# jungmannlab/picasso

Hardware: AMD Instinct MI355X
Metric: localizations/sec (7x7 ROI, MLE) (higher is better)
Workload: dtype f32+f64; 1 GPU; 10000-frame 512x512 uint16 simulated DNA-PAINT movie per GPU, 1001675 spots per GPU, 7x7 ROI MLE (sigmaxy), identify+cut+fit+table resident in HBM; frames=10000, height=512, width=512, box=7, max_it=100, localizations_total=1001675, mle_mode=refit, refit_spots_rank0=7346, frame_ranges_in_flight=2, all_gather=none

## Files before the change

picasso_amd/csrc/fit_common.h:

```cpp
#pragma once
#include <math.h>

#include "pmi_common.h"

namespace pmi {

#ifndef FIT_WAVES_N
#define FIT_WAVES_N 4
#endif
constexpr int FIT_WAVES = FIT_WAVES_N;
constexpr int FIT_NT = FIT_WAVES * PMI_WAVE;
constexpr int FIT_MAXPIX = PMI_MAX_BOX * PMI_MAX_BOX;

struct ConstDiv { float g, r; int fast; };
inline ConstDiv make_const_div(float g)
{
    ConstDiv c;
    c.g = g;
    c.r = (float)(1.0 / (double)g);
    c.fast = (g == g) && fabsf(g) > 1e-15f && fabsf(g) < 1e15f;
    if (g == 1.0f) c.fast = 2;
    return c;
}
__device__ __forceinline__ float div_const(float x, const ConstDiv &c)
// ... 29 lines not shown
    }
}

struct FitParams {
    const float *spots;
    float *spots_out;
    const void *movie;
    const int32_t *frame, *y, *x;
    int dtype;
    int64_t Y, X;
    float baseline, sensitivity, gain;
    ConstDiv gdiv;
    int64_t N;
    const int64_t *d_n;
    int box;
    int libm_glibc;
    double eps;
    int max_it;
    float *thetas, *crlbs, *loglik;
    int32_t *iterations;
    unsigned long long *queue;
    unsigned *strict_queue;
    int64_t first;
    double *fisher;
    float eps_lo, eps_hi;
    int32_t *flag_list;
    unsigned *flag_count;
    unsigned *flag_reasons;
    const int32_t *final_list;
    const unsigned *final_list_n;
    unsigned char *refit_mark;
    float *ng_io;
    unsigned char *accept;
    int crop_y0, crop_x0, crop_cy, crop_cx;
    double min_ng;
    const int32_t *alist;
    const unsigned *alist_n;
    int32_t *alist_out;
    unsigned *alist_blk_out;
};
enum : unsigned { FLAG_MARGIN = 1u, FLAG_CURVATURE = 2u, FLAG_NARROW = 4u, FLAG_SWING = 8u, FLAG_WILD = 16u, FLAG_SLOW = 32u, FLAG_UNSTABLE = 64u };
constexpr int FLAG_REASONS = 7;
constexpr double FIT_UNSTABLE_LMAX = 1.9;
constexpr int FISHER_STRIDE = 21;
enum { FIT_STAGE_NEWTON = 1, FIT_STAGE_FINAL = 2, FIT_STAGE_INIT_ONLY = 4, FIT_STAGE_ITERATE_ONLY = 8 };
constexpr int FIT_SLOW_ITERATIONS = 64;
#ifndef PMI_MARGIN_GROWTH
#define PMI_MARGIN_GROWTH 0.0625f
#endif
constexpr float FIT_MARGIN_GROWTH = PMI_MARGIN_GROWTH;
constexpr float FIT_NARROW_SIGMA = 0.5f;
constexpr float FIT_WOBBLE_RATIO = 0.9f;
constexpr float FIT_WOBBLE_FLOOR = 1.9073486e-6f;
constexpr int FIT_WOBBLE_RUN = 3;
constexpr int FIT_WOBBLE_LATE = 9;
constexpr float FIT_TOP_FLAG = 16.0f;

template <int CTRL, int ROW_MASK = 0xf>
__device__ __forceinline__ float dpp_f(float v)
{
    return __builtin_bit_cast(float, __builtin_amdgcn_update_dpp(0, __builtin_bit_cast(int, v), CTRL, ROW_MASK, 0xf, false));
}
__device__ __forceinline__ float wave_sum(float v)
{
    v += dpp_f<0xB1>(v);
    v += dpp_f<0x4E>(v);
    v += dpp_f<0x141>(v);
    v += dpp_f<0x140>(v);
    v += dpp_f<0x142, 0xA>(v);
    v += dpp_f<0x143, 0xC>(v);
    return __builtin_bit_cast(float, __builtin_amdgcn_readlane(__builtin_bit_cast(int, v), 63));
}
template <int CTRL, int ROW_MASK = 0xf>
__device__ __forceinline__ double dpp_d(double v)
{
    long long b = __builtin_bit_cast(long long, v);
    int lo = (int)(b & 0xffffffffLL), hi = (int)(b >> 32);
    lo = __builtin_amdgcn_update_dpp(0, lo, CTRL, ROW_MASK, 0xf, false);
// ... 68 lines not shown
```

picasso_amd/csrc/gaussmle.hip:

```cpp
#include <algorithm>
#include <cmath>
#include <cstdlib>
#include <cstring>
#include <vector>

#include "fit_common.h"

namespace pmi {

__device__ __forceinline__ unsigned borderline(float D, int kk, float eps_lo, float eps_hi)
{
    const float wide = fmaxf(1.0f, (float)(kk - 1) * FIT_MARGIN_GROWTH);
    const float epsf = 0.5f * (eps_lo + eps_hi), epsm = 0.5f * (eps_hi - eps_lo) * wide;
    return ((D >= epsf - epsm && D < epsf + epsm) ? FLAG_MARGIN : 0u) | (kk > FIT_SLOW_ITERATIONS ? FLAG_SLOW : 0u);
}
struct StepHistory { float prev, prev2, wprev; int run; };
__device__ __forceinline__ bool wobbles(float st, float value, int kk, StepHistory &h)
{
    const float w = kk >= 3 ? (st - 2.0f * h.prev) + h.prev2 : 0.0f;
    const bool wob = w * h.wprev < 0.0f && fabsf(w) > FIT_WOBBLE_RATIO * fabsf(h.wprev) && fabsf(w) > FIT_WOBBLE_FLOOR * fabsf(value);
    h.run = wob ? h.run + 1 : 0;
    h.wprev = w; h.prev2 = h.prev; h.prev = st;
    return h.run >= FIT_WOBBLE_RUN || (h.run >= 2 && kk >= FIT_WOBBLE_LATE);
}
// ... 266 lines not shown
{
    double A[36], V[36];
    bool nonfinite = false;
    for (int i = 0; i < NP * NP; i++) { A[i] = Min[i]; if (!isfinite(A[i])) nonfinite = true; }
    if (nonfinite) { for (int i = 0; i < NP; i++) diag[i] = NAN; return; }
    for (int i = 0; i < NP; i++) for (int j = 0; j < NP; j++) V[i * NP + j] = (i == j) ? 1.0 : 0.0;
    for (int sweep = 0; sweep < 60; sweep++) {
        double off = 0.0;
        for (int a = 0; a < NP; a++) for (int b = a + 1; b < NP; b++) off += A[a * NP + b] * A[a * NP + b];
        if (off == 0.0) break;
        for (int a = 0; a < NP; a++)
            for (int b = a + 1; b < NP; b++) {
                double apq = A[a * NP + b];
                if (apq == 0.0) continue;
                double tau = (A[b * NP + b] - A[a * NP + a]) / (2.0 * apq);
                double tt = (tau >= 0 ? 1.0 : -1.0) / (fabs(tau) + sqrt(1.0 + tau * tau));
                double c = 1.0 / sqrt(1.0 + tt * tt), s = tt * c;
                for (int k = 0; k < NP; k++) { double x = A[k * NP + a], y = A[k * NP + b]; A[k * NP + a] = c * x - s * y; A[k * NP + b] = s * x + c * y; }
                for (int k = 0; k < NP; k++) { double x = A[a * NP + k], y = A[b * NP + k]; A[a * NP + k] = c * x - s * y; A[b * NP + k] = s * x + c * y; }
                for (int k = 0; k < NP; k++) { double x = V[k * NP + a], y = V[k * NP + b]; V[k * NP + a] = c * x - s * y; V[k * NP + b] = s * x + c * y; }
            }
    }
    double smax = 0.0;
    for (int i = 0; i < NP; i++) smax = fmax(smax, fabs(A[i * NP + i]));
    const double cutoff = 1e-15 * smax;
    for (int i = 0; i < NP; i++) {
        double acc = 0.0;
        for (int k = 0; k < NP; k++) { double lam = A[k * NP + k]; if (fabs(lam) > cutoff) acc += V[i * NP + k] * V[i * NP + k] / lam; }
        diag[i] = acc;
    }
}

template <int NP>
__global__ __launch_bounds__(256) void crlb_kernel(const double *__restrict__ fisher, int64_t first, int64_t N,
                                                   const int64_t *__restrict__ d_n, float *__restrict__ crlbs,
                                                   const int32_t *__restrict__ list, const unsigned *__restrict__ list_n,
                                                   int32_t *__restrict__ unstable, unsigned *__restrict__ unstable_n,
                                                   unsigned *__restrict__ reasons, const unsigned char *__restrict__ refit_mark,
                                                   const unsigned char *__restrict__ accept)
{
    int64_t n = N;
    if (d_n) { int64_t dn = *d_n; n = dn < n ? dn : n; }
    int64_t t = (int64_t)blockIdx.x * blockDim.x + threadIdx.x;
    int64_t sidx = first + t;
    if (list) {
        if (t >= (int64_t)*list_n) return;
        sidx = (int64_t)list[t];
        t = sidx - first;
    } else if (sidx >= n) return;
    else if (accept && !accept[sidx]) return;
    const double *f = fisher + t * FISHER_STRIDE;
    double M[36];
    {
        int e = 0;
#pragma unroll
        for (int k = 0; k < NP; k++)
#pragma unroll
            for (int l = k; l < NP; l++) { const double v = f[e++]; M[k * NP + l] = v; M[l * NP + k] = v; }
    }
    if (unstable && !(refit_mark && refit_mark[t])) {
        double dinv[NP], v[NP], lam = 0.0;
        bool ok = true;
#pragma unroll
        for (int i = 0; i < NP; i++) { const double m = M[i * NP + i]; ok = ok && m > 0.0 && m < 1e300; dinv[i] = 1.0 / sqrt(m); v[i] = 1.0 + 0.125 * (double)i; }
        if (ok) {
            double C[NP * NP], C2[NP * NP], t8 = 0.0;
#pragma unroll
            for (int i = 0; i < NP; i++)
#pragma unroll
                for (int k = 0; k < NP; k++) C[i * NP + k] = M[i * NP + k] * dinv[i] * dinv[k];
#pragma unroll
            for (int i = 0; i < NP; i++)
#pragma unroll
                for (int k = i; k < NP; k++) {
                    double a = 0.0;
#pragma unroll
                    for (int q = 0; q < NP; q++) a += C[i * NP + q] * C[q * NP + k];
                    C2[i * NP + k] = a; C2[k * NP + i] = a;
                }
#pragma unroll
            for (int i = 0; i < NP; i++)
#pragma unroll
                for (int k = i; k < NP; k++) {
// ... 43 lines not shown
            if (c == i) { D[i] = a; rD[i] = 1.0 / a; if (!(a > 0.0)) bad = true; }
            else L[i * NP + c] = a * rD[c];
        }
    }
    double Li[36];
#pragma unroll
    for (int i = 0; i < NP; i++)
#pragma unroll
        for (int c = 0; c < NP; c++) Li[i * NP + c] = (i == c) ? 1.0 : 0.0;
#pragma unroll
    for (int c = 0; c < NP; c++)
#pragma unroll
        for (int i = c + 1; i < NP; i++) {
            double a = 0.0;
#pragma unroll
            for (int k = c; k < i; k++) a -= L[i * NP + k] * Li[k * NP + c];
            Li[i * NP + c] = a;
        }
    double trInv = 0.0;
#pragma unroll
    for (int i = 0; i < NP; i++) {
        double a = 0.0;
#pragma unroll
        for (int k = i; k < NP; k++) a += Li[k * NP + i] * Li[k * NP + i] * rD[k];
        diag[i] = a;
        trInv += a;
    }
    if (!(trM * trInv < 1e12)) bad = true;
    if (bad) pinv_diag_jacobi<NP>(M, diag);
    float *co = crlbs + sidx * 6;
#pragma unroll
    for (int l = 0; l < NP; l++) co[l] = (float)diag[l];
    if (NP == 5) co[5] = (float)diag[4];
}

template <int NP, bool FROM_MOVIE>
static void launch_fit_ppl(int ppl, dim3 grid, hipStream_t s, const FitParams &p, int stages)
{
    switch (ppl) {
    case 1: hipLaunchKernelGGL((mle_fit_kernel<NP, 1, FROM_MOVIE>), grid, dim3(FIT_NT), 0, s, p, stages); break;
    case 2: hipLaunchKernelGGL((mle_fit_kernel<NP, 2, FROM_MOVIE>), grid, dim3(FIT_NT), 0, s, p, stages); break;
    case 3: hipLaunchKernelGGL((mle_fit_kernel<NP, 3, FROM_MOVIE>), grid, dim3(FIT_NT), 0, s, p, stages); break;
    case 4: hipLaunchKernelGGL((mle_fit_kernel<NP, 4, FROM_MOVIE>), grid, dim3(FIT_NT), 0, s, p, stages); break;
    case 5: hipLaunchKernelGGL((mle_fit_kernel<NP, 5, FROM_MOVIE>), grid, dim3(FIT_NT), 0, s, p, stages); break;
    case 6: hipLaunchKernelGGL((mle_fit_kernel<NP, 6, FROM_MOVIE>), grid, dim3(FIT_NT), 0, s, p, stages); break;
    default: hipLaunchKernelGGL((mle_fit_kernel<NP, 7, FROM_MOVIE>), grid, dim3(FIT_NT), 0, s, p, stages); break;
    }
}


bool launch_fit_g8(const FitParams &p, int method, bool from_movie, int cu_count, float *state, int stages, hipStream_t s);
void launch_fit_strict(const FitParams &p, int method, bool from_movie, const int32_t *list, const unsigned *list_n,
                       int64_t max_items, int cu_count, hipStream_t s);

constexpr int64_t FIT_BATCH = 1 << 22;
constexpr int ACC_BLOCK = 1024;
__global__ __launch_bounds__(256) void accept_count_kernel(const unsigned char *__restrict__ accept, int64_t first, int64_t N,
                                                           const int64_t *__restrict__ d_n, unsigned *__restrict__ blk_cnt)
{
    int64_t n = N;
    if (d_n) { const int64_t dn = *d_n; n = dn < n ? dn : n; }
    __shared__ unsigned s_c[4];
    const int64_t base = first + (int64_t)blockIdx.x * ACC_BLOCK;
    unsigned c = 0;
#pragma unroll
    for (int q = 0; q < ACC_BLOCK / 256; q++) {
        const int64_t sp = base + q * 256 + threadIdx.x;
        c += (unsigned)__popcll(__ballot(sp < n && accept[sp] != 0));
    }
    if ((threadIdx.x & 63) == 0) s_c[threadIdx.x >> 6] = c;
    __syncthreads();
    if (threadIdx.x == 0) blk_cnt[blockIdx.x] = s_c[0] + s_c[1] + s_c[2] + s_c[3];
}
__global__ __launch_bounds__(1024) void accept_scan_kernel(unsigned *__restrict__ blk, int nblk, unsigned *__restrict__ total)
{
    __shared__ unsigned s_w[16];
    __shared__ unsigned s_carry;
    if (threadIdx.x == 0) s_carry = 0;
    __syncthreads();
    const int lane = threadIdx.x & 63, w = threadIdx.x >> 6;
    for (int b0 = 0; b0 < nblk; b0 += 1024) {
        const int i = b0 + (int)threadIdx.x;
        const unsigned v = i < nblk ? blk[i] : 0u;
        unsigned inc = v;
#pragma unroll
        for (int off = 1; off < 64; off <<= 1) { const unsigned t = __shfl_up(inc, off); if (lane >= off) inc += t; }
        if (lane == 63) s_w[w] = inc;
        __syncthreads();
        unsigned before = s_carry;
// ... 4 lines not shown
        __syncthreads();
    }
    if (threadIdx.x == 0) *total = s_carry;
}
__global__ __launch_bounds__(256) void accept_write_kernel(const unsigned char *__restrict__ accept, int64_t first, int64_t N,
                                                           const int64_t *__restrict__ d_n, const unsigned *__restrict__ blk_off,
                                                           int32_t *__restrict__ alist)
{
    int64_t n = N;
    if (d_n) { const int64_t dn = *d_n; n = dn < n ? dn : n; }
    __shared__ unsigned s_c[ACC_BLOCK / 64];
    const int64_t base = first + (int64_t)blockIdx.x * ACC_BLOCK;
    const int lane = threadIdx.x & 63, w = threadIdx.x >> 6;
    unsigned long long bal[ACC_BLOCK / 256];
#pragma unroll
    for (int q = 0; q < ACC_BLOCK / 256; q++) {
        const int64_t sp = base + q * 256 + threadIdx.x;
        bal[q] = __ballot(sp < n && accept[sp] != 0);
        if (lane == 0) s_c[q * 4 + w] = (unsigned)__popcll(bal[q]);
    }
    __syncthreads();
    const unsigned off0 = blk_off[blockIdx.x];
#pragma unroll
    for (int q = 0; q < ACC_BLOCK / 256; q++) {
        if ((bal[q] >> lane) & 1ull) {
            unsigned off = off0;
            for (int k = 0; k < q * 4 + w; k++) off += s_c[k];
            off += (unsigned)__popcll(bal[q] & ((1ull << lane) - 1ull));
            alist[off] = (int32_t)(base + q * 256 + threadIdx.x);
        }
    }
}
static int build_accept_list(const unsigned char *accept, int64_t first, int64_t N, const int64_t *d_n, unsigned *blk,
                             int32_t *alist, hipStream_t s)
{
    const int64_t count = N - first;
    const int nblk = (int)((count + ACC_BLOCK - 1) / ACC_BLOCK);
    hipLaunchKernelGGL(accept_count_kernel, dim3((unsigned)nblk), dim3(256), 0, s, accept, first, N, d_n, blk);
    hipLaunchKernelGGL(accept_scan_kernel, dim3(1), dim3(1024), 0, s, blk, nblk, blk + nblk);
    hipLaunchKernelGGL(accept_write_kernel, dim3((unsigned)nblk), dim3(256), 0, s, accept, first, N, d_n, (const unsigned *)blk, alist);
    PMI_HIP(hipGetLastError());
    return PMI_OK;
}

static int g_mle_mode = PMI_MLE_REFIT;
static double g_mle_margin = 0.001;
static int g_mle_libm = PMI_LIBM_AUTO;
static thread_local LastFitStats g_mle_stats;

__global__ void zero_words_kernel(unsigned *__restrict__ a, int na, unsigned *__restrict__ b, int nb)
{
    for (int i = threadIdx.x; i < na; i += blockDim.x) a[i] = 0u;
    for (int i = threadIdx.x; i < nb; i += blockDim.x) b[i] = 0u;
}

__global__ void flag_stats_kernel(const unsigned *__restrict__ flag_counts, int64_t nb, unsigned *__restrict__ stats)
{
    unsigned total = 0;
    for (int64_t b = 0; b < nb; b++) total += flag_counts[b];
    stats[0] = total;
}

static int mle_mode_now()
{
    static const char *env = getenv("PMI_MLE_MODE");
    if (env) {
        if (!strcmp(env, "fast")) return PMI_MLE_FAST;
        if (!strcmp(env, "strict")) return PMI_MLE_STRICT;
        if (!strcmp(env, "refit")) return PMI_MLE_REFIT;
    }
    return g_mle_mode;
}
static int mle_libm_now()
{
    static const char *env = getenv("PMI_MLE_LIBM");
    if (env) {
        if (!strcmp(env, "auto")) return PMI_LIBM_AUTO;
        if (!strcmp(env, "glibc")) return PMI_LIBM_GLIBC;
        if (!strcmp(env, "device")) return PMI_LIBM_DEVICE;
    }
    return g_mle_libm;
}

int fit_impl(FitParams p, int method, bool from_movie, int range, hipStream_t s)
{
    if (p.box < 3 || p.box > PMI_MAX_BOX || (p.box & 1) == 0) { set_error("box must be odd, 3..%d (got %d)", PMI_MAX_BOX, p.box); return PMI_ERR_ARG; }
    if (method != PMI_MLE_SIGMA && method != PMI_MLE_SIGMAXY) { set_error("Method not available."); return PMI_ERR_ARG; }
    if (p.N < 0) { set_error("negative N"); return PMI_ERR_ARG; }
    if (p.N == 0) return PMI_OK;
    if (p.N > 0x7fffffffLL) { set_error("too many spots for one call"); return PMI_ERR_ARG; }
    const int g_cu_count = device_cu_count();
    const int mode = mle_mode_now();
    const int64_t BATCH = FIT_BATCH;
    const int64_t nb = (p.N + BATCH - 1) / BATCH;
    void *ptr = nullptr, *fptr = nullptr;
    int rc;
    if ((rc = scratch(SCR_FIT, (size_t)nb * 40 + 64, &ptr)) != PMI_OK) return rc;
    const size_t per_batch = (size_t)std::min<int64_t>(p.N, BATCH);
    const size_t acc_blocks = (per_batch + ACC_BLOCK - 1) / ACC_BLOCK + 2;
    if ((rc = scratch(SCR_STAGE_D, per_batch * (FISHER_STRIDE * sizeof(double) + 12 * sizeof(float) + 3 * sizeof(int32_t) + 1) + acc_blocks * sizeof(unsigned) + 32, &fptr)) != PMI_OK) return rc;
    float *state = reinterpret_cast<float *>((char *)fptr + per_batch * FISHER_STRIDE * sizeof(double));
    int32_t *flag_list = reinterpret_cast<int32_t *>(state + per_batch * 12);
    int32_t *unstable_list = flag_list + per_batch;
    int32_t *acc_list = unstable_list + per_batch;
    unsigned *acc_blk = reinterpret_cast<unsigned *>(acc_list + per_batch);
    unsigned char *refit_mark = reinterpret_cast<unsigned char *>(acc_blk + acc_blocks);
    unsigned long long *queues = (unsigned long long *)ptr;
    unsigned *flag_counts = (unsigned *)(queues + 3 * nb);
    unsigned *strict_queues = flag_counts + 2 * nb;
    void *sptr = nullptr;
    if ((rc = scratch(SCR_STATS, 64, &sptr)) != PMI_OK) return rc;
    unsigned *stats = (unsigned *)sptr;
    hipLaunchKernelGGL(zero_words_kernel, dim3(1), dim3(256), 0, s, (unsigned *)ptr, (int)(nb * 10), stats, 16);
    p.flag_reasons = stats + 1;
    p.fisher = (double *)fptr;
    const int libm = mle_libm_now();
    const bool libm_all = libm != PMI_LIBM_DEVICE;
    p.libm_glibc = libm == PMI_LIBM_GLIBC || (libm == PMI_LIBM_AUTO && p.box <= 5);
    static const char *menv = tuning_env("PMI_MLE_MARGIN");
    const double margin = menv ? atof(menv) : g_mle_margin;
    const double ulp = ldexp(1.0, (int)floor(log2(std::max(1.0, p.box / 2.0))) - 23);
    const double margin_abs = std::max(p.eps * margin, 4.0 * ulp);
    p.eps_lo = (float)(p.eps - margin_abs);
    p.eps_hi = (float)(p.eps + margin_abs);
    const int ppl = (p.box * p.box + 63) / 64;
    const int64_t Ntotal = p.N;
    ScopedKernelTimer tm(s, &g_last_times.fit_ms);
    static const bool force_wave_per_spot = tuning_env("PMI_FIT_WAVE_PER_SPOT") != nullptr;
    const bool g8 = !force_wave_per_spot && p.box <= 15;
    float *cut = nullptr;
    static const bool no_keep = tuning_env("PMI_MLE_NO_KEEP") != nullptr;
    if (g8 && from_movie && mode != PMI_MLE_STRICT && !no_keep) {
        void *cptr = nullptr;
        if ((rc = scratch(SCR_STAGE_C, per_batch * (size_t)(p.box * p.box) * sizeof(float), &cptr)) != PMI_OK) return rc;
        cut = (float *)cptr;
    }
    p.spots_out = nullptr;
    if (p.ng_io && !(g8 && from_movie && cut)) { set_error("deferred exact stage outside the row-per-lane fit"); return PMI_ERR_ARG; }
    for (int64_t bi = 0; bi < nb; bi++) {
        p.first = bi * BATCH;
        p.N = std::min<int64_t>(Ntotal, p.first + BATCH);
        p.flag_list = mode == PMI_MLE_REFIT ? flag_list : nullptr;
        p.flag_count = flag_counts + bi;
        p.strict_queue = strict_queues + bi;
        p.refit_mark = mode == PMI_MLE_REFIT ? refit_mark : nullptr;
        if (p.refit_mark && !g8) PMI_HIP(hipMemsetAsync(refit_mark, 0, (size_t)(p.N - p.first), s));
        const int64_t count = p.N - p.first;
        const int64_t blocks = std::min<int64_t>((count + FIT_WAVES - 1) / FIT_WAVES, (int64_t)g_cu_count * 8);
        const dim3 grid((unsigned)std::max<int64_t>(blocks, 1));
        auto wave_per_spot = [&](int stages) {
            p.queue = queues + 3 * bi + (stages == FIT_STAGE_FINAL ? (p.final_list ? 2 : 1) : 0);
            if (method == PMI_MLE_SIGMAXY) {
                if (from_movie) launch_fit_ppl<6, true>(ppl, grid, s, p, stages); else launch_fit_ppl<6, false>(ppl, grid, s, p, stages);
            } else {
                if (from_movie) launch_fit_ppl<5, true>(ppl, grid, s, p, stages); else launch_fit_ppl<5, false>(ppl, grid, s, p, stages);
            }
        };
        if (mode != PMI_MLE_STRICT && g8 && from_movie && cut) {
            FitParams pi = p;
            pi.spots_out = cut;
            launch_fit_g8(pi, method, true, g_cu_count, state, FIT_STAGE_INIT_ONLY, s);
            PMI_HIP(hipGetLastError());
            FitParams q = p;
            q.spots = cut - p.first * (int64_t)(p.box * p.box);
            if (p.ng_io) {
                int32_t *al = nb == 1 && p.alist_out ? p.alist_out : acc_list;
                unsigned *ab = nb == 1 && p.alist_out ? p.alist_blk_out : acc_blk;
                if ((rc = build_accept_list(p.accept, p.first, p.N, p.d_n, ab, al, s)) != PMI_OK) return rc;
                q.alist = al;
                q.alist_n = ab + (count + ACC_BLOCK - 1) / ACC_BLOCK;
            }
            launch_fit_g8(q, method, false, g_cu_count, state, FIT_STAGE_ITERATE_ONLY, s);
            PMI_HIP(hipGetLastError());
            if (mode == PMI_MLE_REFIT)
                launch_fit_strict(q, method, false, flag_list, q.flag_count, count, g_cu_count, s);
            PMI_HIP(hipGetLastError());
            launch_fit_g8(q, method, false, g_cu_count, state, FIT_STAGE_FINAL, s);
        } else {
        if (mode == PMI_MLE_STRICT) {
            FitParams ps = p;
            ps.libm_glibc = libm_all;
            launch_fit_strict(ps, method, from_movie, nullptr, nullptr, count, g_cu_count, s);
        } else {
            if (g8) launch_fit_g8(p, method, from_movie, g_cu_count, state, FIT_STAGE_NEWTON, s);
            else wave_per_spot(FIT_STAGE_NEWTON);
            PMI_HIP(hipGetLastError());
            if (mode == PMI_MLE_REFIT)
                launch_fit_strict(p, method, from_movie, flag_list, p.flag_count, count, g_cu_count, s);
        }
        PMI_HIP(hipGetLastError());
        if (g8) launch_fit_g8(p, method, from_movie, g_cu_count, state, FIT_STAGE_FINAL, s);
        else wave_per_spot(FIT_STAGE_FINAL);
        }
        PMI_HIP(hipGetLastError());
        const unsigned cb = (unsigned)((count + 255) / 256);
        unsigned *unstable_n = flag_counts + nb + bi;
        auto crlb = [&](const int32_t *list, const unsigned *list_n, int32_t *out, unsigned *out_n) {
            if (method == PMI_MLE_SIGMAXY)
                hipLaunchKernelGGL((crlb_kernel<6>), dim3(cb), dim3(256), 0, s, p.fisher, p.first, p.N, p.d_n, p.crlbs, list, list_n, out, out_n, p.flag_reasons, p.refit_mark, p.accept);
            else
                hipLaunchKernelGGL((crlb_kernel<5>), dim3(cb), dim3(256), 0, s, p.fisher, p.first, p.N, p.d_n, p.crlbs, list, list_n, out, out_n, p.flag_reasons, p.refit_mark, p.accept);
        };
        const bool second = mode == PMI_MLE_REFIT;
        crlb(nullptr, nullptr, second ? unstable_list : nullptr, second ? unstable_n : nullptr);
        PMI_HIP(hipGetLastError());
        if (second) {
            FitParams r = p;
            r.strict_queue = strict_queues + nb + bi;
            if (cut) { r.spots = cut - p.first * (int64_t)(p.box * p.box); }
            const bool r_movie = cut ? false : from_movie;
            launch_fit_strict(r, method, r_movie, unstable_list, unstable_n, count, g_cu_count, s);
            PMI_HIP(hipGetLastError());
            r.final_list = unstable_list; r.final_list_n = unstable_n;
            if (g8) launch_fit_g8(r, method, r_movie, g_cu_count, state, FIT_STAGE_FINAL, s);
            else {
                FitParams keep = p;
                p = r;
                wave_per_spot(FIT_STAGE_FINAL);
                p = keep;
            }
            PMI_HIP(hipGetLastError());
            crlb(unstable_list, unstable_n, nullptr, nullptr);
            PMI_HIP(hipGetLastError());
        }
    }
    hipLaunchKernelGGL(flag_stats_kernel, dim3(1), dim3(1), 0, s, flag_counts, mode == PMI_MLE_REFIT ? 2 * nb : 0, stats);
    PMI_HIP(hipGetLastError());
    if ((rc = g_mle_stats.record(0, range, stats, s)) != PMI_OK) return rc;
    tm.stop();
    return PMI_OK;
}

static int read_last_stats(unsigned (&h)[16], hipStream_t s)
{
    if (g_mle_stats.valid()) PMI_HIP(hipStreamSynchronize(s));
    return g_mle_stats.read(h);
}

__global__ void cut_spots_kernel(const void *__restrict__ movie, int dtype, int64_t Y, int64_t X,
                                 const int32_t *__restrict__ frame, const int32_t *__restrict__ y,
                                 const int32_t *__restrict__ x, int64_t N, const int64_t *__restrict__ d_n,
                                 int box, float baseline, float sensitivity, ConstDiv gdiv, float *__restrict__ spots)
{
    int64_t n = N;
    if (d_n) { int64_t dn = *d_n; n = dn < n ? dn : n; }
    const int npix = box * box, h = box / 2;
    int64_t total = n * npix;
    for (int64_t t = (int64_t)blockIdx.x * blockDim.x + threadIdx.x; t < total; t += (int64_t)gridDim.x * blockDim.x) {
        int64_t i = t / npix;
        int q = (int)(t - i * npix);
        int a = q / box, c = q - a * box;
        float raw = load_movie_px(movie, dtype, ((int64_t)frame[i] * Y + (y[i] - h + a)) * X + (x[i] - h + c));
        spots[t] = div_const((raw - baseline) * sensitivity, gdiv);
    }
}
// ... 315 lines not shown
```

picasso_amd/csrc/gaussmle_g8.hip:

```cpp
#include <algorithm>

#include "fit_common.h"
#include "ng_common.h"

namespace pmi {

__device__ __forceinline__ float sum8(float v)
{
    v += dpp_f<0xB1>(v);
    v += dpp_f<0x4E>(v);
    v += dpp_f<0x141>(v);
    return v;
}
__device__ __forceinline__ float min8(float v)
{
    v = fminf(v, dpp_f<0xB1>(v));
    v = fminf(v, dpp_f<0x4E>(v));
    v = fminf(v, dpp_f<0x141>(v));
    return v;
}
__device__ __forceinline__ double sum8_d(double v)
{
    v += dpp_d<0xB1>(v);
    v += dpp_d<0x4E>(v);
// ... 437 lines not shown
                    for (int c = 0; c < W; c++) { nbt[c] = nb[c]; nbt[(W - 1) * W + c] = nb2[c]; }
                }
                __builtin_amdgcn_wave_barrier();
                __threadfence_block();
                const float vc = nbt[(H + 1) * W + (H + 1)];
                bool fm = true;
                if (rowok) {
#pragma unroll
                    for (int l = 0; l < B; l++) {
                        const float o = nb[l + 1];
                        const bool before = j < H || (j == H && l < H);
                        const bool centre = j == H && l == H;
                        fm = fm && (centre || (before ? vc > o : vc >= o));
                        const float gy = sub_rn(nbt[(j + 2) * W + l + 1], nbt[j * W + l + 1]);
                        const float gx = sub_rn(nb[l + 2], nb[l]);
                        terms[j * B + l] = add_rn(mul_rn(gy, uy[l]), mul_rn(gx, ux[l]));
                    }
                }
                __builtin_amdgcn_wave_barrier();
                __threadfence_block();
                float ng = 0.0f;
#pragma unroll
                for (int q = 0; q < B * B; q++)
                    if (q != H * B + H) ng = add_rn(ng, terms[q]);
                const unsigned long long gm = (GS == 64 ? ~0ull : ((1ull << GS) - 1ull)) << (lane & ~(GS - 1));
                const bool first_max = (__ballot(fm) & gm) == gm;
                if (need) {
                    keep = first_max && (double)ng > p.min_ng;
                    if (j == 0) p.ng_io[sidx] = ng;
                }
                __builtin_amdgcn_wave_barrier();
            }
            if (spot_ok && j == 0) p.accept[sidx] = keep ? 1 : 0;
        }
    }
    if (!loaded) load_row<B, FROM_MOVIE>(p, sidx, j, spot_ok && rowok, d);
    if (FROM_MOVIE && p.spots_out && spot_ok && rowok && keep) {
        float *o = p.spots_out + (sidx - p.first) * (B * B) + j * B;
#pragma unroll
        for (int i = 0; i < B; i++) o[i] = d[i];
    }

    double ps = 0.0, px = 0.0;
#pragma unroll
    for (int i = 0; i < B; i++) { ps += (double)d[i]; px += (double)d[i] * (double)i; }
    double sum = gsum_d<GS>(ps), sx_ = gsum_d<GS>(px), sy_ = gsum_d<GS>(ps * (double)j);
    float fmin_l = INFINITY;
    {
        double t3[B];
#pragma unroll
        for (int i = 0; i < B; i++) {
            double a = (double)d[i];
            if (i > 0) a = (double)d[i - 1] + a;
            if (i + 1 < B) a += (double)d[i + 1];
            t3[i] = a;
        }
        const bool up = j > 0, dn = j + 1 < B;
        const int nrow = 1 + (up ? 1 : 0) + (dn ? 1 : 0);
        const double n2 = (double)(nrow * 2), n3 = (double)(nrow * 3);
        const double r2 = 1.0 / n2, r3 = 1.0 / n3;
#pragma unroll
        for (int i = 0; i < B; i++) {
            const double a = from_prev_d(t3[i]), c = from_next_d(t3[i]);
            double tot = t3[i];
            if (up) tot = a + tot;
            if (dn) tot += c;
// ... 107 lines not shown
                    sidx = p.alist ? (int64_t)p.alist[cand] : cand;
                    const float4 *si = reinterpret_cast<const float4 *>(state + (sidx - p.first) * 12);
                    const float4 s0 = si[0], s1 = si[1], s2 = si[2];
                    th[0] = s0.x; th[1] = s0.y; th[2] = s0.z; th[3] = s0.w; th[4] = s1.x; th[5] = s1.y;
                    ms[0] = s1.z; ms[1] = s1.w; ms[2] = s2.x; ms[3] = s2.y; ms[4] = s2.z; ms[5] = s2.w;
                    load_row<B, FROM_MOVIE>(p, sidx, j, rowok, d);
                    role = make_role<NP, B>(th, ms, j);
                    kk = 0;
                    flags = 0u;
                    active = p.max_it > 0;
                    if (!active && j == 0) {
                        float *to = p.thetas + sidx * 6;
#pragma unroll
                        for (int l = 0; l < 5; l++) to[l] = th[l];
                        to[5] = NP == 6 ? th[5] : th[4];
                        p.iterations[sidx] = 0;
                        sidx = -1;
                    }
                }
            }
            next += __popcll(want);
            if (!__any(active)) {
                if (next >= end) break;
                continue;
            }
        } else if (!any_active) {
            break;
        }
        active = newton_step<NP, B>(d, th, role, xs, j, rowok, active, kk, p.eps, p.max_it, p.eps_lo, p.eps_hi, flags);
    }
}

template <int NP, int B, bool FROM_MOVIE>
__global__ __launch_bounds__(FIT_NT) void g8_final_kernel(FitParams p)
{
    constexpr int GS = GroupOf<B>::GS, NSPW = 64 / GS;
    __shared__ __attribute__((aligned(16))) double s_x[FIT_WAVES][NSPW][GS * 7];
    const int lane = threadIdx.x & 63, wid = threadIdx.x >> 6;
    const int g = lane / GS, j = lane & (GS - 1);
    const bool rowok = j < B;
    const float jf = (float)j;
    int64_t n = p.N;
    if (p.d_n) { int64_t dn = *p.d_n; n = dn < n ? dn : n; }
    int64_t sidx = p.first + ((int64_t)blockIdx.x * FIT_WAVES + wid) * NSPW + g;
    bool spot_ok = sidx < n;
    if (p.final_list) {
        const int64_t w0 = ((int64_t)blockIdx.x * FIT_WAVES + wid) * NSPW, items = (int64_t)*p.final_list_n;
        if (__builtin_amdgcn_readfirstlane((int)(w0 >= items))) return;
        spot_ok = w0 + g < items;
        sidx = spot_ok ? (int64_t)p.final_list[w0 + g] : p.first;
    } else if (__builtin_amdgcn_readfirstlane((int)(p.first + ((int64_t)blockIdx.x * FIT_WAVES + wid) * NSPW >= n))) return;
    else if (p.accept) spot_ok = spot_ok && p.accept[sidx] != 0;

    float d[B], th[6];
    load_row<B, FROM_MOVIE>(p, sidx, j, spot_ok && rowok, d);
#pragma unroll
    for (int l = 0; l < 6; l++) th[l] = spot_ok ? p.thetas[sidx * 6 + l] : 1.f;
    double *red = &s_x[wid][g][0];
    float *cols = reinterpret_cast<float *>(red);
    const float sgy = NP == 6 ? th[5] : th[4];
    const BTerms tx = boundary_terms(jf, th[0], th[4]);
    const BTerms ty = boundary_terms(jf, th[1], sgy);
    {
        float4 *c = reinterpret_cast<float4 *>(cols + j * 12);
        c[0] = make_float4(tx.A * tx.A, tx.A * tx.E, tx.A, tx.A * tx.S);
        c[1] = make_float4(tx.E * tx.E, tx.E, tx.E * tx.S, 1.0f);
        c[2] = make_float4(tx.S, tx.S * tx.S, 0.f, 0.f);
    }
    __builtin_amdgcn_wave_barrier();
    __threadfence_block();
    double T[10];
#pragma unroll
    for (int e = 0; e < 10; e++) T[e] = 0.0;
    float ll_loc = 0.f;
    const float N_ = th[2];
    const float NEy = N_ * ty.E;
#pragma unroll
    for (int i = 0; i < B; i++) {
        const float4 *c = reinterpret_cast<const float4 *>(cols + i * 12);
        const float4 c0 = c[0], c1 = c[1];
        const float2 c2 = *reinterpret_cast<const float2 *>(cols + i * 12 + 8);
        const float model = NEy * c1.y + th[3];
        if (rowok) {
            const double md = (double)model;
            double inv = (double)rcp_f32(model);
            inv = inv * (2.0 - md * inv);
            inv = inv * (2.0 - md * inv);
            T[0] += (double)c0.x * inv; T[1] += (double)c0.y * inv; T[2] += (double)c0.z * inv; T[3] += (double)c0.w * inv;
            T[4] += (double)c1.x * inv; T[5] += (double)c1.y * inv; T[6] += (double)c1.z * inv; T[7] += inv;
            T[8] += (double)c2.x * inv; T[9] += (double)c2.y * inv;
            if (model > 0.f) {
// ... 28 lines not shown
    constexpr int NE_ = NP * (NP + 1) / 2;
    double mine[3] = {0.0, 0.0, 0.0};
#pragma unroll
    for (int r0 = 0; r0 < 21; r0 += 7) {
        if (r0 < NE_) {
#pragma unroll
            for (int e = 0; e < 7; e++) red[j * 7 + e] = Mloc[r0 + e];
            __builtin_amdgcn_wave_barrier();
            __threadfence_block();
#pragma unroll
            for (int t = 0; t < 3; t++) {
                const int e = j + GS * t - r0;
                if (e >= 0 && e < 7) {
                    double acc = 0.0;
#pragma unroll
                    for (int r = 0; r < B; r++) acc += red[r * 7 + e];
                    mine[t] = acc;
                }
            }
            __builtin_amdgcn_wave_barrier();
        }
    }
    double *fo = p.fisher + (sidx - p.first) * FISHER_STRIDE;
    if (spot_ok) {
#pragma unroll
        for (int t = 0; t < 3; t++)
            if (j + GS * t < NE_) fo[j + GS * t] = mine[t];
    }
    const float ll = gsum<GS>(ll_loc);
    if (spot_ok && j == 0) p.loglik[sidx] = ll;
}

template <int NP, int B, bool FROM_MOVIE>
static void launch_g8(const FitParams &p, float *state, int cu_count, int stages, hipStream_t s)
{
    constexpr int NSPW = 64 / GroupOf<B>::GS;
    const int64_t count = p.N - p.first;
    const int64_t waves = (count + NSPW - 1) / NSPW;
    const dim3 flat((unsigned)((waves + FIT_WAVES - 1) / FIT_WAVES));
    const int64_t pw = std::max<int64_t>(1, std::min<int64_t>((int64_t)cu_count * 24, (count + 63) / 64));
    const dim3 pers((unsigned)((pw + FIT_WAVES - 1) / FIT_WAVES));
    if (stages & (FIT_STAGE_NEWTON | FIT_STAGE_INIT_ONLY))
        hipLaunchKernelGGL((g8_init_kernel<NP, B, FROM_MOVIE>), flat, dim3(FIT_NT), 0, s, p, state);
    if (stages & (FIT_STAGE_NEWTON | FIT_STAGE_ITERATE_ONLY))
        hipLaunchKernelGGL((g8_iterate_kernel<NP, B, FROM_MOVIE>), pers, dim3(FIT_NT), 0, s, p, (const float *)state);
    if (stages & FIT_STAGE_FINAL)
        hipLaunchKernelGGL((g8_final_kernel<NP, B, FROM_MOVIE>), flat, dim3(FIT_NT), 0, s, p);
}

template <int NP, bool FROM_MOVIE>
static void launch_g8_box(const FitParams &p, float *state, int cu_count, int stages, hipStream_t s)
{
    switch (p.box) {
    case 3: launch_g8<NP, 3, FROM_MOVIE>(p, state, cu_count, stages, s); break;
    case 5: launch_g8<NP, 5, FROM_MOVIE>(p, state, cu_count, stages, s); break;
    case 7: launch_g8<NP, 7, FROM_MOVIE>(p, state, cu_count, stages, s); break;
    case 9: launch_g8<NP, 9, FROM_MOVIE>(p, state, cu_count, stages, s); break;
    case 11: launch_g8<NP, 11, FROM_MOVIE>(p, state, cu_count, stages, s); break;
    case 13: launch_g8<NP, 13, FROM_MOVIE>(p, state, cu_count, stages, s); break;
    default: launch_g8<NP, 15, FROM_MOVIE>(p, state, cu_count, stages, s); break;
    }
}

bool launch_fit_g8(const FitParams &p, int method, bool from_movie, int cu_count, float *state, int stages, hipStream_t s)
{
    if (p.box > 15) return false;
    if (method == PMI_MLE_SIGMAXY) {
        if (from_movie) launch_g8_box<6, true>(p, state, cu_count, stages, s); else launch_g8_box<6, false>(p, state, cu_count, stages, s);
    } else {
        if (from_movie) launch_g8_box<5, true>(p, state, cu_count, stages, s); else launch_g8_box<5, false>(p, state, cu_count, stages, s);
    }
    return true;
}

}
```

picasso_amd/csrc/identify.hip:

```cpp
#include <algorithm>
#include <cmath>
#include <type_traits>
#include <mutex>
#include <vector>

#include "pmi_common.h"

#pragma clang fp contract(off)

namespace pmi {

static int64_t g_narrow_chunk_frames = 0;

static __device__ __forceinline__ float mul_rn(float a, float b) { return a * b; }
static __device__ __forceinline__ float add_rn(float a, float b) { return a + b; }
static __device__ __forceinline__ float sub_rn(float a, float b) { return a - b; }

constexpr int ID_TH = 32;
constexpr int ID_TW = 128;
constexpr int ID_NT = 256;
constexpr int ID_SHARDS = 8;

struct IdParams {
    int64_t Y, X;
// ... 301 lines not shown
template <typename T>
__global__ __launch_bounds__(256) void narrow_to_u16_kernel(const T *__restrict__ src, long long n, uint16_t *__restrict__ dst,
                                                            int *__restrict__ flag)
{
    bool bad = false;
    for (long long i = ((long long)blockIdx.x * blockDim.x + threadIdx.x) * 4; i < n; i += (long long)gridDim.x * blockDim.x * 4) {
        if (__hip_atomic_load(flag, __ATOMIC_RELAXED, __HIP_MEMORY_SCOPE_AGENT) != 0) return;
        T v[4];
        const bool full = i + 4 <= n;
        if (full) { const uint4 q = *reinterpret_cast<const uint4 *>(src + i); __builtin_memcpy(v, &q, 16); }
        else for (int k = 0; k < 4; k++) v[k] = i + k < n ? src[i + k] : (T)0;
        uint16_t o[4];
#pragma unroll
        for (int k = 0; k < 4; k++) {
            if constexpr (sizeof(T) == 4 && !std::is_integral<T>::value) {
                const float f = (float)v[k];
                bad = bad || !(f >= 0.0f && f <= 65535.0f && f == __builtin_truncf(f));
                o[k] = (uint16_t)(int)f;
            } else if constexpr (std::is_signed<T>::value) {
                bad = bad || v[k] < 0 || v[k] > 65535;
                o[k] = (uint16_t)v[k];
            } else {
                bad = bad || v[k] > 65535u;
                o[k] = (uint16_t)v[k];
            }
        }
        if (full) { uint2 w; w.x = o[0] | ((unsigned)o[1] << 16); w.y = o[2] | ((unsigned)o[3] << 16); *reinterpret_cast<uint2 *>(dst + i) = w; }
        else for (int k = 0; k < 4 && i + k < n; k++) dst[i + k] = o[k];
    }
    if (__any(bad) && (threadIdx.x & 63) == 0) atomicOr(flag, 1);
}


int identify_impl(const void *d_movie, int dtype, int64_t F, int64_t Y, int64_t X, int box, double min_ng,
                  const int64_t *roi4, int64_t f_lo, int64_t f_hi, int64_t label_offset,
                  int32_t *d_frame, int32_t *d_y, int32_t *d_x, float *d_ng, int64_t cap, int64_t *d_out_n,
                  bool defer_exact, hipStream_t s)
{
    if (box < 3 || box > PMI_MAX_BOX || (box & 1) == 0) { set_error("box must be odd, 3..%d (got %d)", PMI_MAX_BOX, box); return PMI_ERR_ARG; }
    if (F < 0 || Y <= 0 || X <= 0 || Y > 65535 || X > 65535) { set_error("bad movie shape (%lld,%lld,%lld)", (long long)F, (long long)Y, (long long)X); return PMI_ERR_ARG; }
    if (cap < 0) { set_error("negative capacity"); return PMI_ERR_ARG; }
    int64_t y0 = 0, x0 = 0, y1 = Y, x1 = X;
    if (roi4) { y0 = roi4[0]; x0 = roi4[1]; y1 = roi4[2]; x1 = roi4[3]; }
    if (y0 < 0 || x0 < 0 || y1 > Y || x1 > X) { set_error("roi outside the frame"); return PMI_ERR_ARG; }
    if (f_lo < 0) f_lo = 0;
    if (f_hi > F - 1) f_hi = F - 1;
    int64_t nf = f_hi - f_lo + 1;
    int64_t cy = y1 - y0, cx = x1 - x0;

    unsigned long long *d_total = nullptr;
    void *ptr = nullptr;
    int rc;
    if ((rc = scratch(SCR_COUNTERS, 256, &ptr)) != PMI_OK) return rc;
    d_total = (unsigned long long *)ptr;
    PMI_HIP(hipMemsetAsync(d_total, 0, 256, s));
    if (nf <= 0 || cy < box + 1 || cx < box + 1) {
        PMI_HIP(hipMemsetAsync(d_out_n, 0, sizeof(int64_t), s));
        return PMI_OK;
    }
    if (nf > 0x7fffffffLL) { set_error("too many frames"); return PMI_ERR_ARG; }

    IdParams p;
    p.Y = Y; p.X = X; p.y0 = (int)y0; p.x0 = (int)x0; p.cy = (int)cy; p.cx = (int)cx;
    p.f_lo = f_lo; p.frame_label_offset = label_offset; p.nframes = (int)nf; p.box = box;
    p.tiles_y = (int)((cy + ID_TH - 1) / ID_TH); p.tiles_x = (int)((cx + ID_TW - 1) / ID_TW);
    p.min_ng = min_ng;

    const float *d_tab = nullptr;
    if ((rc = unit_table(box, &d_tab)) != PMI_OK) return rc;
    Record *recs = nullptr, *grouped = nullptr;
    int *fc = nullptr;
    size_t rec_bytes = (size_t)std::max<int64_t>(cap, 1) * sizeof(Record);
    if ((rc = scratch(SCR_RECORDS, rec_bytes * ID_SHARDS, &ptr)) != PMI_OK) return rc; recs = (Record *)ptr;
    if ((rc = scratch(SCR_RECORDS2, rec_bytes, &ptr)) != PMI_OK) return rc; grouped = (Record *)ptr;
    if ((rc = scratch(SCR_FRAME_COUNT, (size_t)nf * 3 * sizeof(int), &ptr)) != PMI_OK) return rc; fc = (int *)ptr;
    int *count = fc, *base = fc + nf, *cursor = fc + 2 * nf;
    PMI_HIP(hipMemsetAsync(count, 0, (size_t)nf * sizeof(int), s));

    {
        ScopedKernelTimer tm(s, &g_last_times.scan_ms);
        bool fast = false;
        rc = PMI_OK;
        rc = launch_scan_u16_fast(d_movie, dtype, Y, X, p.y0, p.x0, p.cy, p.cx, f_lo, label_offset, p.nframes, box, min_ng,
                                      d_tab, recs, cap, d_total, count, s, &fast, nullptr, defer_exact);
        p.gate = nullptr;
        const bool wide = dtype == PMI_U32 || dtype == PMI_I32 || dtype == PMI_F32;
        static const bool no_narrow = tuning_env("PMI_IDENTIFY_NO_NARROW") != nullptr;
        if (rc == PMI_OK && !fast && wide && !no_narrow) {
            rc = launch_scan_u16_fast(d_movie, dtype, Y, X, p.y0, p.x0, p.cy, p.cx, f_lo, label_offset, p.nframes, box, min_ng,
                                      d_tab, recs, cap, d_total, count, s, &fast, nullptr, false, (const float *)d_movie, 0);
        }
        if (rc == PMI_OK && !fast && wide && !no_narrow && ((uintptr_t)d_movie & 15) == 0 && ((Y * X) & 3) == 0) {
            const int64_t frame_px = Y * X;
            const int64_t chunk = g_narrow_chunk_frames > 0 ? g_narrow_chunk_frames : std::max<int64_t>(1, ((int64_t)1 << 29) / frame_px);
            const int64_t nchunks = (nf + chunk - 1) / chunk;
            void *tmp = nullptr, *gptr = nullptr;
            if ((rc = scratch(SCR_NARROW, (size_t)std::min<int64_t>(nf, chunk) * frame_px * 2 + 64, &tmp)) != PMI_OK) return rc;
            if ((rc = scratch(SCR_GATES, (size_t)nchunks * sizeof(int), &gptr)) != PMI_OK) return rc;
            int *gates = (int *)gptr;
            PMI_HIP(hipMemsetAsync(gates, 0, (size_t)nchunks * sizeof(int), s));
            bool all_fast = true;
            for (int64_t ci = 0; ci < nchunks && rc == PMI_OK; ci++) {
                const int64_t c0 = ci * chunk, n = std::min<int64_t>(chunk, nf - c0);
                const long long npx = (long long)n * frame_px;
                const unsigned nb = (unsigned)std::min<long long>((npx / 4 + 255) / 256, 256 * 32);
                const char *srcp = (const char *)d_movie + (size_t)(f_lo + c0) * frame_px * 4;
                if (dtype == PMI_F32) hipLaunchKernelGGL(narrow_to_u16_kernel<float>, dim3(nb), dim3(256), 0, s, (const float *)srcp, npx, (uint16_t *)tmp, gates + ci);
                else if (dtype == PMI_I32) hipLaunchKernelGGL(narrow_to_u16_kernel<int32_t>, dim3(nb), dim3(256), 0, s, (const int32_t *)srcp, npx, (uint16_t *)tmp, gates + ci);
                else hipLaunchKernelGGL(narrow_to_u16_kernel<uint32_t>, dim3(nb), dim3(256), 0, s, (const uint32_t *)srcp, npx, (uint16_t *)tmp, gates + ci);
                PMI_HIP(hipGetLastError());
// ... 191 lines not shown
```

Before: 377.8 million localizations/s.

## Cut launches and shrink grids for refit list kernels and accept counting

Several launch-count and grid-size reductions across the fit pipeline. The init kernel now counts accepted spots per block with wave ballots and atomics, so build_accept_list can skip its separate count kernel. The refit final-pass and CRLB list kernels become grid-stride kernels launched with about one workgroup per CU rather than a full-size grid over mostly empty work. In identify, two memsets are merged into one zeroing kernel. Together these are meant to cut fixed per-launch and empty-block overhead on the small refit path, at the cost of extra atomics in the init kernel.

```diff
diff --git a/picasso_amd/csrc/fit_common.h b/picasso_amd/csrc/fit_common.h
--- a/picasso_amd/csrc/fit_common.h
+++ b/picasso_amd/csrc/fit_common.h
@@ -85,6 +85,7 @@
     unsigned char *refit_mark;
     float *ng_io;
     unsigned char *accept;
+    unsigned *accept_cnt;
     int crop_y0, crop_x0, crop_cy, crop_cx;
     double min_ng;
     const int32_t *alist;
@@ -96,7 +97,11 @@
 constexpr int FLAG_REASONS = 7;
 constexpr double FIT_UNSTABLE_LMAX = 1.9;
 constexpr int FISHER_STRIDE = 21;
+constexpr int ACC_BLOCK = 1024;
 enum { FIT_STAGE_NEWTON = 1, FIT_STAGE_FINAL = 2, FIT_STAGE_INIT_ONLY = 4, FIT_STAGE_ITERATE_ONLY = 8 };
+constexpr int FINAL_LIST_WG_PER_CU = 1;
+constexpr int CRLB_LIST_WG_PER_CU = 1;
+constexpr int CRLB_LIST_NT = 64;
 constexpr int FIT_SLOW_ITERATIONS = 64;
 #ifndef PMI_MARGIN_GROWTH
 #define PMI_MARGIN_GROWTH 0.0625f
diff --git a/picasso_amd/csrc/gaussmle.hip b/picasso_amd/csrc/gaussmle.hip
--- a/picasso_amd/csrc/gaussmle.hip
+++ b/picasso_amd/csrc/gaussmle.hip
@@ -322,23 +322,10 @@
 }
 
 template <int NP>
-__global__ __launch_bounds__(256) void crlb_kernel(const double *__restrict__ fisher, int64_t first, int64_t N,
-                                                   const int64_t *__restrict__ d_n, float *__restrict__ crlbs,
-                                                   const int32_t *__restrict__ list, const unsigned *__restrict__ list_n,
-                                                   int32_t *__restrict__ unstable, unsigned *__restrict__ unstable_n,
-                                                   unsigned *__restrict__ reasons, const unsigned char *__restrict__ refit_mark,
-                                                   const unsigned char *__restrict__ accept)
-{
-    int64_t n = N;
-    if (d_n) { int64_t dn = *d_n; n = dn < n ? dn : n; }
-    int64_t t = (int64_t)blockIdx.x * blockDim.x + threadIdx.x;
-    int64_t sidx = first + t;
-    if (list) {
-        if (t >= (int64_t)*list_n) return;
-        sidx = (int64_t)list[t];
-        t = sidx - first;
-    } else if (sidx >= n) return;
-    else if (accept && !accept[sidx]) return;
+__device__ __forceinline__ void crlb_spot(const double *__restrict__ fisher, int64_t t, int64_t sidx, float *__restrict__ crlbs,
+                                          int32_t *__restrict__ unstable, unsigned *__restrict__ unstable_n,
+                                          unsigned *__restrict__ reasons, const unsigned char *__restrict__ refit_mark)
+{
     const double *f = fisher + t * FISHER_STRIDE;
     double M[36];
     {
@@ -448,6 +435,33 @@
 #pragma unroll
     for (int l = 0; l < NP; l++) co[l] = (float)diag[l];
     if (NP == 5) co[5] = (float)diag[4];
+}
+
+template <int NP>
+__global__ __launch_bounds__(256) void crlb_kernel(const double *__restrict__ fisher, int64_t first, int64_t N,
+                                                   const int64_t *__restrict__ d_n, float *__restrict__ crlbs,
+                                                   int32_t *__restrict__ unstable, unsigned *__restrict__ unstable_n,
+                                                   unsigned *__restrict__ reasons, const unsigned char *__restrict__ refit_mark,
+                                                   const unsigned char *__restrict__ accept)
+{
+    int64_t n = N;
+    if (d_n) { int64_t dn = *d_n; n = dn < n ? dn : n; }
+    const int64_t t = (int64_t)blockIdx.x * blockDim.x + threadIdx.x;
+    const int64_t sidx = first + t;
+    if (sidx >= n) return;
+    if (accept && !accept[sidx]) return;
+    crlb_spot<NP>(fisher, t, sidx, crlbs, unstable, unstable_n, reasons, refit_mark);
+}
+template <int NP>
+__global__ __launch_bounds__(CRLB_LIST_NT) void crlb_list_kernel(const double *__restrict__ fisher, int64_t first,
+                                                                float *__restrict__ crlbs, const int32_t *__restrict__ list,
+                                                                const unsigned *__restrict__ list_n)
+{
+    const int64_t items = (int64_t)*list_n, stride = (int64_t)gridDim.x * blockDim.x;
+    for (int64_t e = (int64_t)blockIdx.x * blockDim.x + threadIdx.x; e < items; e += stride) {
+        const int64_t sidx = (int64_t)list[e];
+        crlb_spot<NP>(fisher, sidx - first, sidx, crlbs, nullptr, nullptr, nullptr, nullptr);
+    }
 }
 
 template <int NP, bool FROM_MOVIE>
@@ -470,7 +484,6 @@
                        int64_t max_items, int cu_count, hipStream_t s);
 
 constexpr int64_t FIT_BATCH = 1 << 22;
-constexpr int ACC_BLOCK = 1024;
 __global__ __launch_bounds__(256) void accept_count_kernel(const unsigned char *__restrict__ accept, int64_t first, int64_t N,
                                                            const int64_t *__restrict__ d_n, unsigned *__restrict__ blk_cnt)
 {
@@ -541,11 +554,11 @@
     }
 }
 static int build_accept_list(const unsigned char *accept, int64_t first, int64_t N, const int64_t *d_n, unsigned *blk,
-                             int32_t *alist, hipStream_t s)
+                             int32_t *alist, hipStream_t s, bool counted = false)
 {
     const int64_t count = N - first;
     const int nblk = (int)((count + ACC_BLOCK - 1) / ACC_BLOCK);
-    hipLaunchKernelGGL(accept_count_kernel, dim3((unsigned)nblk), dim3(256), 0, s, accept, first, N, d_n, blk);
+    if (!counted) hipLaunchKernelGGL(accept_count_kernel, dim3((unsigned)nblk), dim3(256), 0, s, accept, first, N, d_n, blk);
     hipLaunchKernelGGL(accept_scan_kernel, dim3(1), dim3(1024), 0, s, blk, nblk, blk + nblk);
     hipLaunchKernelGGL(accept_write_kernel, dim3((unsigned)nblk), dim3(256), 0, s, accept, first, N, d_n, (const unsigned *)blk, alist);
     PMI_HIP(hipGetLastError());
@@ -557,10 +570,11 @@
 static int g_mle_libm = PMI_LIBM_AUTO;
 static thread_local LastFitStats g_mle_stats;
 
-__global__ void zero_words_kernel(unsigned *__restrict__ a, int na, unsigned *__restrict__ b, int nb)
+__global__ void zero_words_kernel(unsigned *__restrict__ a, int na, unsigned *__restrict__ b, int nb, unsigned *__restrict__ c, int nc)
 {
     for (int i = threadIdx.x; i < na; i += blockDim.x) a[i] = 0u;
     for (int i = threadIdx.x; i < nb; i += blockDim.x) b[i] = 0u;
+    for (int i = threadIdx.x; i < nc; i += blockDim.x) c[i] = 0u;
 }
 
 __global__ void flag_stats_kernel(const unsigned *__restrict__ flag_counts, int64_t nb, unsigned *__restrict__ stats)
@@ -620,7 +634,10 @@
     void *sptr = nullptr;
     if ((rc = scratch(SCR_STATS, 64, &sptr)) != PMI_OK) return rc;
     unsigned *stats = (unsigned *)sptr;
-    hipLaunchKernelGGL(zero_words_kernel, dim3(1), dim3(256), 0, s, (unsigned *)ptr, (int)(nb * 10), stats, 16);
+    const bool g8_counts = p.ng_io && nb == 1;
+    unsigned *const cnt_blk = p.alist_out ? p.alist_blk_out : acc_blk;
+    hipLaunchKernelGGL(zero_words_kernel, dim3(1), dim3(256), 0, s, (unsigned *)ptr, (int)(nb * 10), stats, 16,
+                       cnt_blk, g8_counts ? (int)((per_batch + ACC_BLOCK - 1) / ACC_BLOCK) : 0);
     p.flag_reasons = stats + 1;
     p.fisher = (double *)fptr;
     const int libm = mle_libm_now();
@@ -668,6 +685,7 @@
         if (mode != PMI_MLE_STRICT && g8 && from_movie && cut) {
             FitParams pi = p;
             pi.spots_out = cut;
+            pi.accept_cnt = g8_counts ? cnt_blk : nullptr;
             launch_fit_g8(pi, method, true, g_cu_count, state, FIT_STAGE_INIT_ONLY, s);
             PMI_HIP(hipGetLastError());
             FitParams q = p;
@@ -675,7 +693,7 @@
             if (p.ng_io) {
                 int32_t *al = nb == 1 && p.alist_out ? p.alist_out : acc_list;
                 unsigned *ab = nb == 1 && p.alist_out ? p.alist_blk_out : acc_blk;
-                if ((rc = build_accept_list(p.accept, p.first, p.N, p.d_n, ab, al, s)) != PMI_OK) return rc;
+                if ((rc = build_accept_list(p.accept, p.first, p.N, p.d_n, ab, al, s, g8_counts)) != PMI_OK) return rc;
                 q.alist = al;
                 q.alist_n = ab + (count + ACC_BLOCK - 1) / ACC_BLOCK;
             }
@@ -704,14 +722,21 @@
         PMI_HIP(hipGetLastError());
         const unsigned cb = (unsigned)((count + 255) / 256);
         unsigned *unstable_n = flag_counts + nb + bi;
-        auto crlb = [&](const int32_t *list, const unsigned *list_n, int32_t *out, unsigned *out_n) {
+        auto crlb = [&](int32_t *out, unsigned *out_n) {
             if (method == PMI_MLE_SIGMAXY)
-                hipLaunchKernelGGL((crlb_kernel<6>), dim3(cb), dim3(256), 0, s, p.fisher, p.first, p.N, p.d_n, p.crlbs, list, list_n, out, out_n, p.flag_reasons, p.refit_mark, p.accept);
+                hipLaunchKernelGGL((crlb_kernel<6>), dim3(cb), dim3(256), 0, s, p.fisher, p.first, p.N, p.d_n, p.crlbs, out, out_n, p.flag_reasons, p.refit_mark, p.accept);
             else
-                hipLaunchKernelGGL((crlb_kernel<5>), dim3(cb), dim3(256), 0, s, p.fisher, p.first, p.N, p.d_n, p.crlbs, list, list_n, out, out_n, p.flag_reasons, p.refit_mark, p.accept);
+                hipLaunchKernelGGL((crlb_kernel<5>), dim3(cb), dim3(256), 0, s, p.fisher, p.first, p.N, p.d_n, p.crlbs, out, out_n, p.flag_reasons, p.refit_mark, p.accept);
+        };
+        auto crlb_list = [&](const int32_t *list, const unsigned *list_n) {
+            const unsigned lb = (unsigned)std::min<int64_t>((count + CRLB_LIST_NT - 1) / CRLB_LIST_NT, (int64_t)g_cu_count * CRLB_LIST_WG_PER_CU);
+            if (method == PMI_MLE_SIGMAXY)
+                hipLaunchKernelGGL((crlb_list_kernel<6>), dim3(lb), dim3(CRLB_LIST_NT), 0, s, p.fisher, p.first, p.crlbs, list, list_n);
+            else
+                hipLaunchKernelGGL((crlb_list_kernel<5>), dim3(lb), dim3(CRLB_LIST_NT), 0, s, p.fisher, p.first, p.crlbs, list, list_n);
         };
         const bool second = mode == PMI_MLE_REFIT;
-        crlb(nullptr, nullptr, second ? unstable_list : nullptr, second ? unstable_n : nullptr);
+        crlb(second ? unstable_list : nullptr, second ? unstable_n : nullptr);
         PMI_HIP(hipGetLastError());
         if (second) {
             FitParams r = p;
@@ -729,7 +754,7 @@
                 p = keep;
             }
             PMI_HIP(hipGetLastError());
-            crlb(unstable_list, unstable_n, nullptr, nullptr);
+            crlb_list(unstable_list, unstable_n);
             PMI_HIP(hipGetLastError());
         }
     }
diff --git a/picasso_amd/csrc/gaussmle_g8.hip b/picasso_amd/csrc/gaussmle_g8.hip
--- a/picasso_amd/csrc/gaussmle_g8.hip
+++ b/picasso_amd/csrc/gaussmle_g8.hip
@@ -493,6 +493,11 @@
                 __builtin_amdgcn_wave_barrier();
             }
             if (spot_ok && j == 0) p.accept[sidx] = keep ? 1 : 0;
+            if (p.accept_cnt) {
+                static_assert(ACC_BLOCK % NSPW == 0, "a wavefront's spots must not straddle two blocks");
+                const unsigned kept = (unsigned)__popcll(__ballot(spot_ok && j == 0 && keep));
+                if (lane == 0 && kept) atomicAdd(p.accept_cnt + (sidx - p.first) / ACC_BLOCK, kept);
+            }
         }
     }
     if (!loaded) load_row<B, FROM_MOVIE>(p, sidx, j, spot_ok && rowok, d);
@@ -666,31 +671,15 @@
 }
 
 template <int NP, int B, bool FROM_MOVIE>
-__global__ __launch_bounds__(FIT_NT) void g8_final_kernel(FitParams p)
-{
-    constexpr int GS = GroupOf<B>::GS, NSPW = 64 / GS;
-    __shared__ __attribute__((aligned(16))) double s_x[FIT_WAVES][NSPW][GS * 7];
-    const int lane = threadIdx.x & 63, wid = threadIdx.x >> 6;
-    const int g = lane / GS, j = lane & (GS - 1);
+__device__ __forceinline__ void g8_final_spots(const FitParams &p, int64_t sidx, bool spot_ok, int j, double *red)
+{
+    constexpr int GS = GroupOf<B>::GS;
     const bool rowok = j < B;
     const float jf = (float)j;
-    int64_t n = p.N;
-    if (p.d_n) { int64_t dn = *p.d_n; n = dn < n ? dn : n; }
-    int64_t sidx = p.first + ((int64_t)blockIdx.x * FIT_WAVES + wid) * NSPW + g;
-    bool spot_ok = sidx < n;
-    if (p.final_list) {
-        const int64_t w0 = ((int64_t)blockIdx.x * FIT_WAVES + wid) * NSPW, items = (int64_t)*p.final_list_n;
-        if (__builtin_amdgcn_readfirstlane((int)(w0 >= items))) return;
-        spot_ok = w0 + g < items;
-        sidx = spot_ok ? (int64_t)p.final_list[w0 + g] : p.first;
-    } else if (__builtin_amdgcn_readfirstlane((int)(p.first + ((int64_t)blockIdx.x * FIT_WAVES + wid) * NSPW >= n))) return;
-    else if (p.accept) spot_ok = spot_ok && p.accept[sidx] != 0;
-
     float d[B], th[6];
     load_row<B, FROM_MOVIE>(p, sidx, j, spot_ok && rowok, d);
 #pragma unroll
     for (int l = 0; l < 6; l++) th[l] = spot_ok ? p.thetas[sidx * 6 + l] : 1.f;
-    double *red = &s_x[wid][g][0];
     float *cols = reinterpret_cast<float *>(red);
     const float sgy = NP == 6 ? th[5] : th[4];
     const BTerms tx = boundary_terms(jf, th[0], th[4]);
@@ -785,6 +774,38 @@
 }
 
 template <int NP, int B, bool FROM_MOVIE>
+__global__ __launch_bounds__(FIT_NT) void g8_final_kernel(FitParams p)
+{
+    constexpr int GS = GroupOf<B>::GS, NSPW = 64 / GS;
+    __shared__ __attribute__((aligned(16))) double s_x[FIT_WAVES][NSPW][GS * 7];
+    const int lane = threadIdx.x & 63, wid = threadIdx.x >> 6;
+    const int g = lane / GS, j = lane & (GS - 1);
+    int64_t n = p.N;
+    if (p.d_n) { int64_t dn = *p.d_n; n = dn < n ? dn : n; }
+    const int64_t sidx = p.first + ((int64_t)blockIdx.x * FIT_WAVES + wid) * NSPW + g;
+    bool spot_ok = sidx < n;
+    if (__builtin_amdgcn_readfirstlane((int)(p.first + ((int64_t)blockIdx.x * FIT_WAVES + wid) * NSPW >= n))) return;
+    if (p.accept) spot_ok = spot_ok && p.accept[sidx] != 0;
+    g8_final_spots<NP, B, FROM_MOVIE>(p, sidx, spot_ok, j, &s_x[wid][g][0]);
+}
+
+template <int NP, int B, bool FROM_MOVIE>
+__global__ __launch_bounds__(FIT_NT) void g8_final_list_kernel(FitParams p)
+{
+    constexpr int GS = GroupOf<B>::GS, NSPW = 64 / GS;
+    __shared__ __attribute__((aligned(16))) double s_x[FIT_WAVES][NSPW][GS * 7];
+    const int lane = threadIdx.x & 63, wid = threadIdx.x >> 6;
+    const int g = lane / GS, j = lane & (GS - 1);
+    const int64_t items = (int64_t)*p.final_list_n, stride = (int64_t)gridDim.x * FIT_WAVES * NSPW;
+    for (int64_t w0 = ((int64_t)blockIdx.x * FIT_WAVES + wid) * NSPW; w0 < items; w0 += stride) {
+        const bool spot_ok = w0 + g < items;
+        const int64_t sidx = spot_ok ? (int64_t)p.final_list[w0 + g] : p.first;
+        g8_final_spots<NP, B, FROM_MOVIE>(p, sidx, spot_ok, j, &s_x[wid][g][0]);
+        __builtin_amdgcn_wave_barrier();
+    }
+}
+
+template <int NP, int B, bool FROM_MOVIE>
 static void launch_g8(const FitParams &p, float *state, int cu_count, int stages, hipStream_t s)
 {
     constexpr int NSPW = 64 / GroupOf<B>::GS;
@@ -797,7 +818,10 @@
         hipLaunchKernelGGL((g8_init_kernel<NP, B, FROM_MOVIE>), flat, dim3(FIT_NT), 0, s, p, state);
     if (stages & (FIT_STAGE_NEWTON | FIT_STAGE_ITERATE_ONLY))
         hipLaunchKernelGGL((g8_iterate_kernel<NP, B, FROM_MOVIE>), pers, dim3(FIT_NT), 0, s, p, (const float *)state);
-    if (stages & FIT_STAGE_FINAL)
+    if ((stages & FIT_STAGE_FINAL) && p.final_list) {
+        const dim3 few((unsigned)std::min<int64_t>(flat.x, (int64_t)cu_count * FINAL_LIST_WG_PER_CU));
+        hipLaunchKernelGGL((g8_final_list_kernel<NP, B, FROM_MOVIE>), few, dim3(FIT_NT), 0, s, p);
+    } else if (stages & FIT_STAGE_FINAL)
         hipLaunchKernelGGL((g8_final_kernel<NP, B, FROM_MOVIE>), flat, dim3(FIT_NT), 0, s, p);
 }
 
diff --git a/picasso_amd/csrc/identify.hip b/picasso_amd/csrc/identify.hip
--- a/picasso_amd/csrc/identify.hip
+++ b/picasso_amd/csrc/identify.hip
@@ -357,6 +357,14 @@
 }
 
 
+__global__ __launch_bounds__(256) void zero_scan_counters_kernel(unsigned *__restrict__ total, int n_total,
+                                                                 int *__restrict__ count, int64_t nf)
+{
+    const int64_t t0 = (int64_t)blockIdx.x * blockDim.x + threadIdx.x, stride = (int64_t)gridDim.x * blockDim.x;
+    for (int64_t i = t0; i < n_total; i += stride) total[i] = 0u;
+    for (int64_t i = t0; i < nf; i += stride) count[i] = 0;
+}
+
 int identify_impl(const void *d_movie, int dtype, int64_t F, int64_t Y, int64_t X, int box, double min_ng,
                   const int64_t *roi4, int64_t f_lo, int64_t f_hi, int64_t label_offset,
                   int32_t *d_frame, int32_t *d_y, int32_t *d_x, float *d_ng, int64_t cap, int64_t *d_out_n,
@@ -378,7 +386,6 @@
     int rc;
     if ((rc = scratch(SCR_COUNTERS, 256, &ptr)) != PMI_OK) return rc;
     d_total = (unsigned long long *)ptr;
-    PMI_HIP(hipMemsetAsync(d_total, 0, 256, s));
     if (nf <= 0 || cy < box + 1 || cx < box + 1) {
         PMI_HIP(hipMemsetAsync(d_out_n, 0, sizeof(int64_t), s));
         return PMI_OK;
@@ -400,7 +407,8 @@
     if ((rc = scratch(SCR_RECORDS2, rec_bytes, &ptr)) != PMI_OK) return rc; grouped = (Record *)ptr;
     if ((rc = scratch(SCR_FRAME_COUNT, (size_t)nf * 3 * sizeof(int), &ptr)) != PMI_OK) return rc; fc = (int *)ptr;
     int *count = fc, *base = fc + nf, *cursor = fc + 2 * nf;
-    PMI_HIP(hipMemsetAsync(count, 0, (size_t)nf * sizeof(int), s));
+    hipLaunchKernelGGL(zero_scan_counters_kernel, dim3((unsigned)std::min<int64_t>((nf + 255) / 256, 64)), dim3(256), 0, s,
+                       (unsigned *)d_total, 64, count, nf);
 
     {
         ScopedKernelTimer tm(s, &g_last_times.scan_ms);
```

Result: slower. 367.1 million localizations/s (-2.8%).
